# ktzsh/object-tracking

Measured on AMD Instinct MI355X. Metric: frames/sec detect+track @416x416, higher is better.
Workload: dtype f32; 1 GPU; BASELINE.json configs[2]: MultiObjDetTracker (YOLOv2 C=12 + ConvLSTM2D(512) + 1x1 + decode/NMS + track ids), 48 clips x 30 frames per GPU per step, 416x416 uint8; the synthetic head is calibrated to 32 CANDIDATE boxes per frame, of which about 20 survive NMS (config.boxes_per_frame: measured).  The step computes the model's TRACKING output, the one MultiObjDetTracker.predict reads (MultiObjDetTrac; parallelism=clip-shard x1

## Files before the change

object_tracking_amd/csrc/dt_internal.h:

```cpp
#pragma once
#include <hip/hip_runtime.h>

#include <atomic>
#include <cstdint>
#include <cstdio>
#include <map>
#include <mutex>
#include <functional>
#include <string>
#include <type_traits>
#include <vector>

#include "../../include/mi355_dt.h"

struct PerDeviceOnce {
    std::atomic<unsigned long long> mask{0};
    std::mutex mu;
    template <class F> int ensure(int *dev_out, F &&setup)
    {
        int dev = -1;
        if (hipGetDevice(&dev) != hipSuccess || dev < 0 || dev > 63) return 1;
        if (dev_out) *dev_out = dev;
        if ((mask.load(std::memory_order_acquire) >> dev) & 1ull) return 0;
        std::lock_guard<std::mutex> lk(mu);
        if ((mask.load(std::memory_order_acquire) >> dev) & 1ull) return 0;
        const int rc = setup(dev);
        if (rc == 0) mask.fetch_or(1ull << dev, std::memory_order_release);
        return rc;
    }
};

typedef float f32x4 __attribute__((ext_vector_type(4)));
typedef float f32x16 __attribute__((ext_vector_type(16)));

enum { ORD_LINEAR = 0, ORD_QUAD = 1 };
enum { EPI_PLAIN = 0, EPI_POOL = 1, EPI_POOL_BOTH = 2, EPI_S2D = 3, EPI_GATES = 4, EPI_PARTIAL = 5 };

struct ConvArgs {
    const float *in;
    long long in_bs;
    int in_ld;
    const float *wt;
    const float *bias;
    float *out;
    long long out_bs;
    int out_ld;
    float *out2;
    int out2_ld;
    const float *xproj;
    long long xp_bs;
    int xp_ld;
    float *cstate;
    long long c_bs;
    int c_ld;
    int B, H, W, Cin, N, M, K;
    int npad;
    float slope;
    int act;
    const float *zeros;
    int ksplit;
    int tile_gn;
    int zbatch;
    long long z_in, z_wt, z_out;
    int force_cfg;
    unsigned *amax_out;
};

enum { CFG_128x128 = 0, CFG_128x64 = 1, CFG_256x128 = 2, CFG_256x256 = 3, CFG_64x128 = 4 };

int launch_conv_igemm(hipStream_t st, const ConvArgs &a, int ks, int order, int epi, int cfg);
int launch_splitk_reduce(hipStream_t st, const float *slab, int S, long long M, int N, const float *bias, float slope,
                         float *out, int out_ld);

void pack_conv_weights(const float *hwio, int ks, int cin_src, int cout_src, const int *cin_map,
                       int cin_dst, const int *n_map, int npad, const float *scale, float *dst);

struct WinoArgs {
    int B, H, W, th, tw, Mt, ts;
    int g;
    const float *in;
    long long in_bs;
    int in_ld, C;
    float *v;
    unsigned short *v_s3;
    int Mp;
    int nt;
    const unsigned *amax;
    unsigned *amax_out;
    const float *m;
    int m_ld, N;
    const float *bias;
    const float *bias16;
    float slope;
    float *out;
    long long out_bs;
    int out_ld;
    float *out2;
    int out2_ld;
    const float *xproj;
    long long xp_bs;
    int xp_ld;
    float *cstate;
    long long c_bs;
    int c_ld;
};
struct Wino4FusedArgs {
    const float *in;
    long long in_bs;
    int in_ld;
    int B, H, W, Cin, N;
    const float *u;
    const float *bias;
    float slope;
    float *out;
    long long out_bs;
    int out_ld;
    float *out2;
    int out2_ld;
    int nby, nbx;
    const float *zeros;
    unsigned *amax_out;
};
int launch_wino4s_fused(hipStream_t st, const Wino4FusedArgs &a, const float *zeros);
void wino4s_fused_pack(const float *u36, int npad, int cin, int cout, float *dst);
struct Conv3H2Args {
    const float *in;
    long long in_bs;
    int in_ld;
    int B, H, W, Cin, N, Np;
    const unsigned short *w;
    const float *pscale;
    const unsigned *amax;
    const float *bias;
    float slope;
    float *out;
    long long out_bs;
    int out_ld;
    float *out2;
    int out2_ld;
    const float *zeros;
    unsigned *amax_out;
    int tiles_x, tiles_y;
    const unsigned short *w1;
    const float *pscale1;
    const float *bias1;
    int N1, Np1;
    float slope1;
};
int launch_conv3_h2(hipStream_t st, const Conv3H2Args &a);
bool conv3_h2_usable(const Conv3H2Args &a);
double conv3_h2_flops(const Conv3H2Args &a);
struct GemmS3Args {
    const unsigned short *a;
    const float *a_f32;
    int a_ld;
    const unsigned short *b;
    float *c;
    long long c_ps;
    int P, Mt, Mp, N, Np, K, ldc;
    const unsigned short *ones, *bias_s3;
    int act;
    float slope;
// ... 329 lines not shown
```

object_tracking_amd/csrc/network.hip:

```cpp
#include <algorithm>
#include <cmath>
#include <cstdarg>
#include <cstdlib>
#include <cstring>
#include <thread>

#include "dt_internal.h"

static const float BN_EPS = 1e-3f;
static const float LEAKY = 0.1f;
static char g_static_err[512] = "";

static const int TRUNK[20][5] = {
    {1, 3, 3, 32, 1},      {2, 3, 32, 64, 1},     {3, 3, 64, 128, 0},    {4, 1, 128, 64, 0},
    {5, 3, 64, 128, 1},    {6, 3, 128, 256, 0},   {7, 1, 256, 128, 0},   {8, 3, 128, 256, 1},
    {9, 3, 256, 512, 0},   {10, 1, 512, 256, 0},  {11, 3, 256, 512, 0},  {12, 1, 512, 256, 0},
    {13, 3, 256, 512, 1},  {14, 3, 512, 1024, 0}, {15, 1, 1024, 512, 0}, {16, 3, 512, 1024, 0},
    {17, 1, 1024, 512, 0}, {18, 3, 512, 1024, 0}, {19, 3, 1024, 1024, 0}, {20, 3, 1024, 1024, 0}};

static inline int round_up(int v, int m) { return (v + m - 1) / m * m; }

int dt_fail(dt_ctx *ctx, int code, const char *fmt, ...)
{
    char buf[512];
// ... 681 lines not shown
    }
    if (consumed) *consumed = off;
    graphs_clear(ctx);
    ctx->det_loaded = true;
    if (const int rc = streams_fresh(ctx)) return rc;
    return build_merged_xproj(ctx);
}

enum { DF_IGEMM = 0, DF_FUSED = 1, DF_S3 = 2, DF_CONV1 = 3, DF_C3H2 = 4 };
static const char *const k_direct_form[] = {"conv_direct_form", "conv_direct_form_fused", "conv_direct_form_s3", "conv_direct_form_conv1", "conv_direct_form_c3h2"};
static void prof_direct_form(dt_ctx *ctx, double flops, double bytes, int family = DF_IGEMM)
{
    if (!ctx->prof) return;
    ProfEntry &e = ctx->prof_tab[k_direct_form[family]];
    e.flops += flops;
    e.bytes += bytes;
}

static const int S3_MINK = 128;
static const long long C3H2_MIN_BLOCKS = 1024;

static bool wino_runs(const dt_ctx *ctx, const WinoWeights &wts, int B, int H, int W, int N)
{
    if (!wts.u) return false;
    const int ts = wts.ts, cin = wts.cin;
    const long long mt = (long long)B * ((H + ts - 1) / ts) * ((W + ts - 1) / ts);
    if (mt >= (1ll << 31) / 64) return false;
    if (4.0 * (ts + 2) * (ts + 2) * (double)mt * ((double)cin + N) > ctx->pol.wino_ws_gb * 1e9) return false;
    const int mint = ctx->pol.wino_mint;
    return ctx->pol.wino == 2 || mt >= (mint > 0 ? mint : (ts == 2 ? 256 : (ts == 4 ? 16 : 32)));
}

static double small_gemm_cost(int Mt, int N, int P, int *cfg_out)
{
    const long long t128 = (long long)P * ((Mt + 127) / 128) * ((N + 127) / 128);
    const long long t64n = (long long)P * ((Mt + 127) / 128) * ((N + 63) / 64);
    const long long t64m = (long long)P * ((Mt + 63) / 64) * ((N + 127) / 128);
    const long long t256 = (long long)P * ((Mt + 255) / 256) * ((N + 255) / 256);
    double best = (double)((t128 + 255) / 256);
    int cfg = CFG_128x128;
    const double c64n = N % 64 == 0 ? (double)((t64n + 255) / 256) * 0.5 / 0.92 : 1e30;
    const double c64m = (double)((t64m + 255) / 256) * 0.5 / 0.92;
    const double c256 = N % 256 == 0 ? (double)((t256 + 255) / 256) * 4.0 / 1.03 : 1e30;
    if (c64n < best) { best = c64n; cfg = CFG_128x64; }
    if (c64m < best) { best = c64m; cfg = CFG_64x128; }
    if (c256 < best) { best = c256; cfg = CFG_256x256; }
    if (cfg_out) *cfg_out = cfg;
    return best;
}

static int pick_cfg_gemm(int Mt, int N, int P)
{
    const long long t128 = (long long)P * ((Mt + 127) / 128) * ((N + 127) / 128);
    if (t128 <= 4096) {
        int cfg;
        (void)small_gemm_cost(Mt, N, P, &cfg);
        return cfg;
    }
    if (N % 256 == 0) {
        const long long t256 = (long long)P * ((Mt + 255) / 256) * (N / 256);
        const double e256 = (double)Mt / (((Mt + 255) / 256) * 256.0) * (double)t256 / (double)(((t256 + 255) / 256) * 256);
        const double e128 = (double)Mt / (((Mt + 127) / 128) * 128.0) * (double)t128 / (double)(((t128 + 511) / 512) * 512);
        if (e256 * 1.03 > e128) return CFG_256x256;
    }
    return CFG_128x128;
}

static int launch_igemm(dt_ctx *ctx, ConvArgs &a, int ks, int order, int epi, int cfg)
{
    a.force_cfg = ctx->pol.conv_cfg >= 0 ? ctx->pol.conv_cfg + 1 : 0;
    return launch_conv_igemm(ctx->stream, a, ks, order, epi, cfg);
}

struct WinoIO {
    const float *in; long long in_bs; int in_ld;
    float *out; long long out_bs; int out_ld;
    float *out2; int out2_ld;
    const float *xproj; long long xp_bs; int xp_ld;
    float *cstate; long long c_bs; int c_ld;
    const float *bias16;
    unsigned *amax_out;
};

struct WinoGeom { int g, th, tw, Mt; };
static WinoGeom wino_geometry(const dt_ctx *ctx, int ts, int B, int H, int W, bool pooled)
{
    WinoGeom q;
    q.g = 1;
    const int g_env = ctx->pol.mosaic;
    double best = (double)((H + ts - 1) / ts) * ((W + ts - 1) / ts);
    for (int g = 2; g <= 4 && !pooled && g_env != 1; ++g) {
        const double t = (double)((g * (H + 1) + ts - 1) / ts) * ((g * (W + 1) + ts - 1) / ts) / (g * g);
        if ((t < best * 0.97 && B >= g * g) || g_env == g) { best = t; q.g = g; }
    }
    if (q.g == 1) { q.th = (H + ts - 1) / ts; q.tw = (W + ts - 1) / ts; q.Mt = B * q.th * q.tw; }
    else {
        q.th = (q.g * (H + 1) + ts - 1) / ts; q.tw = (q.g * (W + 1) + ts - 1) / ts;
        q.Mt = ((B + q.g * q.g - 1) / (q.g * q.g)) * q.th * q.tw;
    }
    return q;
}

struct Leaves { const float *lo[2]; long long floats[2]; int next, cols; };
static Leaves conv_leaves(int epi, const float *out, int out_ld, const float *out2, int out2_ld, long long M, int cout)
{
    return Leaves{{out, out2}, {(epi == EPI_POOL || epi == EPI_S2D ? M / 4 : M) * out_ld, out2 ? M / 4 * out2_ld : 0}, epi == EPI_POOL_BOTH ? 1 : 0,
                  epi == EPI_S2D ? 4 * cout : cout};
}
static void amax_forget(dt_ctx *ctx, const Leaves &lv) { amax_forget(ctx, lv.lo[0], lv.floats[0]); amax_forget(ctx, lv.lo[1], lv.floats[1]); }
static void amax_note(dt_ctx *ctx, const Leaves &lv, int slot) { amax_note(ctx, lv.lo[lv.next], lv.floats[lv.next], lv.cols, slot); }

struct WinoChoice { WinoGeom q; int nt; };
static WinoChoice choose_wino(const dt_ctx *ctx, const WinoWeights &wts, int N, int B, int H, int W, bool pooled, bool gates)
{
    const int ts = wts.ts, cin = wts.cin;
    WinoChoice c{wino_geometry(ctx, ts, B, H, W, pooled), 0};
    const bool rec = ts == 4 && gates;
    const bool h2_avail = h2_wanted(ctx) && wts.h2;
    const int minrows = h2_avail ? ctx->pol.s3_minrows_h2 : ctx->pol.s3_minrows, rec_minrows = h2_avail ? ctx->pol.s3_rec_minrows_h2 : ctx->pol.s3_rec_minrows;
    if (((ts == 6 && !gates) || rec) && ctx->pol.s3 != 0 && cin % 32 == 0 && N % 128 == 0 && wts.npad % 128 == 0 && wino_gemm_s3_usable(c.q.Mt, cin, N) &&
        (ctx->pol.s3 == 2 || (cin >= S3_MINK && (rec ? (rec_minrows > 0 && c.q.Mt >= rec_minrows) : c.q.Mt >= minrows))) && wts.s3)
        c.nt = h2_avail ? 2 : 3;
    return c;
}
static WinoChoice choose_wino(const dt_ctx *ctx, const WinoWeights &wts, int N, int B, int H, int W, const WinoIO &io) { return choose_wino(ctx, wts, N, B, H, W, io.out2 != nullptr, io.cstate != nullptr); }

static int run_wino(dt_ctx *ctx, const WinoWeights &wts, const WinoChoice &wc, const float *bias, int N, int B, int H, int W, const WinoIO &io, float slope,
                    const char *tag, int cin_alg = 0 ,
                    int in_slot = AMAX_TEST )
{
    const int ts = wts.ts, cin = wts.cin, npad = wts.npad;
    const double cin_df = cin_alg > 0 ? cin_alg : cin;
    amax_forget(ctx, io.out ? conv_leaves(io.out2 ? EPI_POOL_BOTH : EPI_PLAIN, io.out, io.out_ld, io.out2, io.out2_ld, (long long)B * H * W, N)
                            : conv_leaves(EPI_POOL, io.out2, io.out2_ld, nullptr, 0, (long long)B * H * W, N));
    WinoArgs w{};
    w.B = B; w.H = H; w.W = W; w.ts = ts;
    w.g = wc.q.g; w.th = wc.q.th; w.tw = wc.q.tw; w.Mt = wc.q.Mt;
    prof_count(ctx, "wino_mosaic:g%d_ts%d", w.g, ts);
    const int P = (ts + 2) * (ts + 2);
    const size_t mt = (size_t)w.Mt;
    const bool h2 = wc.nt == 2;
    const unsigned short *u_s3 = h2 ? wts.h2.get() : (wc.nt == 3 ? wts.s3.get() : nullptr);
    const int NT = h2 ? 2 : 3;
    const size_t mp = (mt + 255) / 256 * 256;
    float *V = ws_get(ctx, "wino_v", u_s3 ? (size_t)P * NT * mp * cin * sizeof(unsigned short) : P * mt * cin * sizeof(float));
    float *Mp = ws_get(ctx, "wino_m", P * mt * N * sizeof(float));
    if (!V || !Mp) return DT_ERR_DEVICE;
    if (u_s3) { w.v_s3 = reinterpret_cast<unsigned short *>(V); w.Mp = (int)mp; }
    const unsigned *amax = nullptr;
    if (h2) {
        amax = in_slot == AMAX_ONE ? amax_slot(ctx, AMAX_ONE) : ensure_amax(ctx, io.in, (long long)B * H * W, cin, io.in_ld, in_slot);
        if (!amax) return DT_ERR_DEVICE;
        w.nt = 2; w.amax = amax;
    }
    w.in = io.in; w.in_bs = io.in_bs; w.in_ld = io.in_ld; w.C = cin; w.v = V;
    w.m = Mp; w.m_ld = N; w.N = N; w.bias = bias; w.bias16 = io.bias16; w.slope = slope;
    w.out = io.out; w.out_bs = io.out_bs; w.out_ld = io.out_ld; w.out2 = io.out2; w.out2_ld = io.out2_ld;
    w.xproj = io.xproj; w.xp_bs = io.xp_bs; w.xp_ld = io.xp_ld;
    w.cstate = io.cstate; w.c_bs = io.c_bs; w.c_ld = io.c_ld;
    {
        ProfScope ps(ctx, "wino_input", 0.0, 4.0 * (double)B * H * W * cin + (u_s3 ? 2.0 * NT : 4.0) * (double)P * mt * cin, tag);
        const int rc = launch_wino_input(ctx->stream, w);
        if (rc) return dt_fail(ctx, launch_code(rc), "%s: Winograd input transform launch failed", tag);
    }
    const double df_flops = 2.0 * B * H * W * 9.0 * cin_df * N;
    const double df_bytes = 4.0 * ((double)B * H * W * cin_df + 9.0 * cin_df * N + (io.out ? (double)B * H * W * N : 0.0) +
                                   (io.out2 ? (double)B * H * W * N / 4.0 : 0.0) + (io.cstate ? 4.0 * B * H * W * N / 4.0 : 0.0));
    if (u_s3) {
        GemmS3Args g{};
        g.a = w.v_s3; g.b = u_s3; g.c = Mp; g.c_ps = (long long)mt * N; g.P = P; g.Mt = w.Mt; g.Mp = (int)mp; g.N = N; g.Np = npad;
        g.K = cin; g.ldc = N; g.half = ctx->pol.s3_half;
        if (h2) { g.nt = 2; g.pscale = wts.h2_pscale.get(); g.amax = amax; }
        ProfScope ps(ctx, "conv_gemm_s3", wino_gemm_s3_flops(g), (double)P * (2.0 * NT * mt * cin + 2.0 * NT * (double)cin * N + 4.0 * (double)mt * N), tag);
        prof_count(ctx, h2 ? "s3_form:f16x2" : "s3_form:bf16x3");
        prof_direct_form(ctx, df_flops, df_bytes, DF_S3);
        if (ps.on) prof_count(ctx, wino_gemm_s3_half_chosen(g, 0) ? "s3_tile:128x2" : "s3_tile:256");
        const int rc = launch_wino_gemm_s3(ctx->stream, g, 0);
        if (rc) return dt_fail(ctx, launch_code(rc), "%s: split-bf16 Winograd GEMM launch failed (rc=%d)", tag, rc);
    } else {
        ConvArgs a{};
        a.in = V; a.in_ld = cin; a.in_bs = (long long)mt * cin;
        a.wt = wts.u.get(); a.bias = nullptr;
        a.out = Mp; a.out_ld = N; a.out_bs = (long long)mt * N;
        a.B = 1; a.H = 1; a.W = w.Mt; a.Cin = cin; a.N = N; a.M = w.Mt; a.K = cin;
        a.npad = npad; a.slope = 1.0f;
        a.zbatch = P; a.z_in = (long long)mt * cin; a.z_wt = (long long)npad * cin; a.z_out = (long long)mt * N;
        ProfScope ps(ctx, "conv_igemm", 2.0 * P * mt * (double)cin * N, 4.0 * P * ((double)mt * cin + (double)cin * N + (double)mt * N), tag);
        prof_direct_form(ctx, df_flops, df_bytes);
        const int rc = launch_igemm(ctx, a, 1, ORD_LINEAR, EPI_PLAIN, pick_cfg_gemm(w.Mt, N, P));
        if (rc) return dt_fail(ctx, launch_code(rc), "%s: Winograd GEMM launch failed (rc=%d)", tag, rc);
    }
    {
        const double outb = (io.out ? (double)B * H * W * N : 0.0) + (io.out2 ? (double)B * H * W * N / 4.0 : 0.0) +
                            (io.cstate ? 3.0 * B * H * W * N / 4.0 + (double)B * H * W * N : 0.0);
        ProfScope ps(ctx, "wino_output", 0.0, 4.0 * ((double)P * mt * N + outb), tag);
        w.amax_out = io.amax_out;
        if (!wino_output_fills_amax(w, io.cstate != nullptr)) w.amax_out = nullptr;
        const int rc = launch_wino_output(ctx->stream, w, io.cstate != nullptr);
        if (rc) return dt_fail(ctx, launch_code(rc), "%s: Winograd output transform launch failed", tag);
    }
    return DT_OK;
}

struct Dest { float *p; int ld; };

static int pick_cfg(int M, int cout, int ks)
{
    if (cout <= 64) return CFG_128x64;
    if (ks == 3 && cout % 256 == 0) {
        const long long t256 = (long long)((M + 255) / 256) * (cout / 256);
        const long long t128 = (long long)((M + 127) / 128) * (cout / 128);
        const double e256 = (double)t256 / (double)(((t256 + 255) / 256) * 256);
        const double e128 = (double)t128 / (double)(((t128 + 511) / 512) * 512);
        if (e256 * 1.05 > e128) return CFG_256x256;
    }
    if (ks == 1 && cout >= 128 && (long long)((M + 255) / 256) * ((cout + 127) / 128) >= 4096) return CFG_256x128;
    return CFG_128x128;
}

static bool s3_1x1_eligible(const dt_ctx *ctx, const ConvLayer &L, long long M)
// ... 1307 lines not shown
```

object_tracking_amd/csrc/winograd.hip:

```cpp
#include <thread>

#include "dt_internal.h"

#define WINO_THREADS 256

template <int V> struct VecOf;
template <> struct VecOf<1> { typedef float T; };
template <> struct VecOf<2> { typedef float T __attribute__((ext_vector_type(2))); };
template <> struct VecOf<4> { typedef float T __attribute__((ext_vector_type(4))); };

template <int V> __device__ __forceinline__ typename VecOf<V>::T vload(const float *p)
{
    return *reinterpret_cast<const typename VecOf<V>::T *>(p);
}
template <int V> __device__ __forceinline__ void vstore(float *p, typename VecOf<V>::T v)
{
    *reinterpret_cast<typename VecOf<V>::T *>(p) = v;
}
template <int V> __device__ __forceinline__ typename VecOf<V>::T vload_nt(const float *p)
{
    return __builtin_nontemporal_load(reinterpret_cast<const typename VecOf<V>::T *>(p));
}
template <int V> __device__ __forceinline__ void vstore_nt(float *p, typename VecOf<V>::T v)
{
    __builtin_nontemporal_store(v, reinterpret_cast<typename VecOf<V>::T *>(p));
}
template <int V> __device__ __forceinline__ float lane_of(const typename VecOf<V>::T &v, int e) { return v[e]; }
template <> __device__ __forceinline__ float lane_of<1>(const float &v, int) { return v; }
template <int V> __device__ __forceinline__ void set_lane(typename VecOf<V>::T &v, int e, float x) { v[e] = x; }
template <> __device__ __forceinline__ void set_lane<1>(float &v, int, float x) { v = x; }
template <int V> __device__ __forceinline__ typename VecOf<V>::T vzero()
{
    typename VecOf<V>::T z;
#pragma unroll
    for (int e = 0; e < V; ++e) set_lane<V>(z, e, 0.0f);
    return z;
}

template <int TS, typename T> __device__ __forceinline__ void bt_1d(T *d)
{
    if (TS == 2) {
        const T t0 = d[0] - d[2], t1 = d[1] + d[2], t2 = d[2] - d[1], t3 = d[1] - d[3];
        d[0] = t0; d[1] = t1; d[2] = t2; d[3] = t3;
    } else if (TS == 6) {
        const T t0 = d[0] - d[6] + 5.25f * (d[4] - d[2]);
        const T t7 = d[7] - d[1] + 5.25f * (d[3] - d[5]);
        const T a = d[2] - 4.25f * d[4] + d[6], b = d[1] - 4.25f * d[3] + d[5];
        const T c = 0.25f * d[2] - 1.25f * d[4] + d[6], e = 0.5f * d[1] - 2.5f * d[3] + 2.0f * d[5];
        const T f = 4.0f * d[2] - 5.0f * d[4] + d[6], g = 2.0f * d[1] - 2.5f * d[3] + 0.5f * d[5];
        d[0] = t0; d[1] = a + b; d[2] = a - b; d[3] = c + e; d[4] = c - e; d[5] = f + g; d[6] = f - g; d[7] = t7;
    } else {
        const T t0 = 4.0f * d[0] - 5.0f * d[2] + d[4];
        const T t1 = -4.0f * (d[1] + d[2]) + d[3] + d[4];
        const T t2 = 4.0f * (d[1] - d[2]) - d[3] + d[4];
        const T t3 = 2.0f * (d[3] - d[1]) - d[2] + d[4];
        const T t4 = 2.0f * (d[1] - d[3]) - d[2] + d[4];
        const T t5 = 4.0f * d[1] - 5.0f * d[3] + d[5];
        d[0] = t0; d[1] = t1; d[2] = t2; d[3] = t3; d[4] = t4; d[5] = t5;
    }
}
template <int TS, typename T> __device__ __forceinline__ void at_1d(T *m)
{
    if (TS == 2) {
        const T y0 = m[0] + m[1] + m[2], y1 = m[1] - m[2] - m[3];
        m[0] = y0; m[1] = y1;
    } else if (TS == 6) {
        const T p1 = m[1] + m[2], q1 = m[1] - m[2], p2 = m[3] + m[4], q2 = m[3] - m[4], p3 = m[5] + m[6], q3 = m[5] - m[6];
        const T y0 = m[0] + p1 + p2 + p3;
        const T y1 = q1 + 2.0f * q2 + 0.5f * q3;
        const T y2 = p1 + 4.0f * p2 + 0.25f * p3;
        const T y3 = q1 + 8.0f * q2 + 0.125f * q3;
        const T y4 = p1 + 16.0f * p2 + 0.0625f * p3;
        const T y5 = q1 + 32.0f * q2 + 0.03125f * q3 + m[7];
        m[0] = y0; m[1] = y1; m[2] = y2; m[3] = y3; m[4] = y4; m[5] = y5;
    } else {
        const T a = m[1] + m[2], b = m[1] - m[2], c = m[3] + m[4], e = m[3] - m[4];
        const T y0 = m[0] + a + c;
        const T y1 = b + 2.0f * e;
        const T y2 = a + 4.0f * c;
        const T y3 = b + 8.0f * e + m[5];
        m[0] = y0; m[1] = y1; m[2] = y2; m[3] = y3;
    }
}

struct TileId {
    int grp, ty, tx;
};
__device__ __forceinline__ TileId tile_id(const WinoArgs &p, int tile)
{
    const int tpf = p.th * p.tw;
    TileId t;
    t.grp = tile / tpf;
    const int r = tile - t.grp * tpf;
    t.ty = r / p.tw;
    t.tx = r - t.ty * p.tw;
    return t;
}
__device__ __forceinline__ bool vpixel(const WinoArgs &p, int grp, int vh, int vw, int &b, int &h, int &w)
{
    if (vh < 0 || vw < 0) return false;
    if (p.g == 1) {
        b = grp; h = vh; w = vw;
        return vh < p.H && vw < p.W;
    }
    const int fy = vh / (p.H + 1), fx = vw / (p.W + 1);
    h = vh - fy * (p.H + 1);
    w = vw - fx * (p.W + 1);
    b = (grp * p.g + fy) * p.g + fx;
    return fy < p.g && fx < p.g && h < p.H && w < p.W && b < p.B;
}

typedef __bf16 wino_bf4 __attribute__((ext_vector_type(4)));
typedef unsigned int wino_u2 __attribute__((ext_vector_type(2)));
__device__ __forceinline__ void s3_split4(const VecOf<4>::T x, wino_u2 t[3])
{
    const wino_bf4 h = __builtin_convertvector(x, wino_bf4);
    const VecOf<4>::T r1 = x - __builtin_convertvector(h, VecOf<4>::T);
    const wino_bf4 m = __builtin_convertvector(r1, wino_bf4);
    const VecOf<4>::T r2 = r1 - __builtin_convertvector(m, VecOf<4>::T);
    const wino_bf4 l = __builtin_convertvector(r2, wino_bf4);
    t[0] = __builtin_bit_cast(wino_u2, h); t[1] = __builtin_bit_cast(wino_u2, m); t[2] = __builtin_bit_cast(wino_u2, l);
}

template <typename T> __device__ __forceinline__ void s3_store(unsigned short *p, const T &v)
{
    __builtin_nontemporal_store(v, reinterpret_cast<T *>(p));
}

typedef _Float16 wino_h4 __attribute__((ext_vector_type(4)));
__device__ __forceinline__ void h2_split4(const VecOf<4>::T x, wino_u2 t[2])
{
    const wino_h4 h = __builtin_convertvector(x, wino_h4);
    const VecOf<4>::T r = x - __builtin_convertvector(h, VecOf<4>::T);
    t[0] = __builtin_bit_cast(wino_u2, h);
    t[1] = __builtin_bit_cast(wino_u2, __builtin_convertvector(r, wino_h4));
}

template <int TS, int V, bool S3 = false> __global__ __launch_bounds__(WINO_THREADS) void wino_input_kernel(WinoArgs p)
{
    static_assert(!S3 || V == 4, "the split-bf16 store is written for float4 items");
    typedef typename VecOf<V>::T T;
    constexpr int NI = TS + 2;
    const int cq_n = p.C / V;
    const long long items = (long long)p.Mt * cq_n;
    const long long plane = (long long)p.Mt * p.C;
    for (long long it = (long long)blockIdx.x * blockDim.x + threadIdx.x; it < items;
         it += (long long)gridDim.x * blockDim.x) {
        int tile, c;
        if constexpr (S3) {
            constexpr int GPB = 16 / V;
            const long long tb = it / GPB;
            c = (int)(tb / p.Mt) * 16 + (int)(it - tb * GPB) * V;
            tile = (int)(tb % p.Mt);
        } else {
            tile = (int)(it / cq_n);
            c = (int)(it - (long long)tile * cq_n) * V;
        }
        const TileId t = tile_id(p, tile);
        T d[NI][NI];
#pragma unroll
        for (int i = 0; i < NI; ++i) {
#pragma unroll
            for (int j = 0; j < NI; ++j) {
                int b, h, w;
                const bool ok = vpixel(p, t.grp, TS * t.ty - 1 + i, TS * t.tx - 1 + j, b, h, w);
                d[i][j] = ok ? vload<V>(p.in + (long long)b * p.in_bs + (long long)(h * p.W + w) * p.in_ld + c) : vzero<V>();
            }
        }
#pragma unroll
        for (int j = 0; j < NI; ++j) {
            T col[NI];
#pragma unroll
            for (int i = 0; i < NI; ++i) col[i] = d[i][j];
            bt_1d<TS>(col);
#pragma unroll
            for (int i = 0; i < NI; ++i) d[i][j] = col[i];
        }
        if constexpr (S3) {
            const long long term = (long long)(p.C >> 4) * p.Mp * 16;
            unsigned short *dst = p.v_s3 + ((long long)(c >> 4) * p.Mp + tile) * 16 + (c & 15);
#pragma unroll
            for (int i = 0; i < NI; ++i) {
                bt_1d<TS>(d[i]);
                wino_u2 tr[NI][3];
#pragma unroll
                for (int j = 0; j < NI; ++j) s3_split4(d[i][j], tr[j]);
#pragma unroll
                for (int j = 0; j < NI; ++j)
#pragma unroll
                    for (int k = 0; k < 3; ++k) s3_store(dst + ((long long)(NI * i + j) * 3 + k) * term, tr[j][k]);
            }
        } else {
            float *dst = p.v + (long long)tile * p.C + c;
#pragma unroll
            for (int i = 0; i < NI; ++i) {
                bt_1d<TS>(d[i]);
#pragma unroll
                for (int j = 0; j < NI; ++j) vstore_nt<V>(dst + (long long)(NI * i + j) * plane, d[i][j]);
            }
        }
    }
}

__device__ __forceinline__ float wino_leaky(float v, float slope) { return v > 0.0f ? v : v * slope; }
__device__ __forceinline__ float wino_hard_sigmoid(float x)
{
    const float y = __fmaf_rn(0.2f, x, 0.5f);
    return fminf(fmaxf(y, 0.0f), 1.0f);
}

template <int TS, int V>
__device__ __forceinline__ void wino_at_m_a(const float *src, long long plane, typename VecOf<V>::T (*m)[TS + 2])
{
    typedef typename VecOf<V>::T T;
    constexpr int NI = TS + 2;
#pragma unroll
    for (int i = 0; i < NI; ++i)
#pragma unroll
        for (int j = 0; j < NI; ++j) m[i][j] = vload_nt<V>(src + (long long)(NI * i + j) * plane);
#pragma unroll
    for (int j = 0; j < NI; ++j) {
        T col[NI];
#pragma unroll
        for (int i = 0; i < NI; ++i) col[i] = m[i][j];
        at_1d<TS>(col);
#pragma unroll
        for (int i = 0; i < TS; ++i) m[i][j] = col[i];
    }
#pragma unroll
    for (int i = 0; i < TS; ++i) at_1d<TS>(m[i]);
}

__device__ __forceinline__ int wino_border_case(const WinoArgs &p, int h, int w)
{
    return (h == 0 ? 1 : 0) | (h == p.H - 1 ? 2 : 0) | (w == 0 ? 4 : 0) | (w == p.W - 1 ? 8 : 0);
}

template <int TS, int V> __global__ __launch_bounds__(WINO_THREADS) void wino_output_kernel(WinoArgs p)
{
    typedef typename VecOf<V>::T T;
    constexpr int NI = TS + 2;
    const int nq = p.N / V;
    const long long items = (long long)p.Mt * nq;
    const long long plane = (long long)p.Mt * p.m_ld;
    float am = 0.0f;
    const bool am_full = p.amax_out && !p.out2, am_pool = p.amax_out && p.out2;
    for (long long it = (long long)blockIdx.x * blockDim.x + threadIdx.x; it < items;
         it += (long long)gridDim.x * blockDim.x) {
        const int tile = (int)(it / nq);
        const int c = (int)(it - (long long)tile * nq) * V;
        const TileId t = tile_id(p, tile);
        T m[NI][NI];
        wino_at_m_a<TS, V>(p.m + (long long)tile * p.m_ld + c, plane, m);
        const T bv = p.bias ? vload<V>(p.bias + c) : vzero<V>();
#pragma unroll
        for (int i = 0; i < TS; ++i)
#pragma unroll
            for (int j = 0; j < TS; ++j) {
                T v = m[i][j] + bv;
#pragma unroll
                for (int e = 0; e < V; ++e) set_lane<V>(v, e, wino_leaky(lane_of<V>(v, e), p.slope));
                m[i][j] = v;
            }
        if (p.out) {
#pragma unroll
            for (int i = 0; i < TS; ++i)
#pragma unroll
                for (int j = 0; j < TS; ++j) {
                    int b, h, w;
                    if (vpixel(p, t.grp, TS * t.ty + i, TS * t.tx + j, b, h, w)) {
                        T v = m[i][j];
                        if (p.bias16) {
                            const int k = wino_border_case(p, h, w);
                            if (k) v = v + vload<V>(p.bias16 + (long long)k * p.N + c);
                        }
                        if (am_full) {
#pragma unroll
                            for (int e = 0; e < V; ++e) am = fmaxf(am, fabsf(lane_of<V>(v, e)));
                        }
                        vstore_nt<V>(p.out + (long long)b * p.out_bs + (long long)(h * p.W + w) * p.out_ld + c, v);
                    }
                }
        }
        if (p.out2) {
            const int H2 = p.H >> 1, W2 = p.W >> 1;
#pragma unroll
            for (int i = 0; i < TS / 2; ++i)
#pragma unroll
                for (int j = 0; j < TS / 2; ++j) {
                    const int h2 = (TS / 2) * t.ty + i, w2 = (TS / 2) * t.tx + j;
                    if (h2 < H2 && w2 < W2) {
                        T mx;
#pragma unroll
                        for (int e = 0; e < V; ++e)
                            set_lane<V>(mx, e, fmaxf(fmaxf(lane_of<V>(m[2 * i][2 * j], e), lane_of<V>(m[2 * i][2 * j + 1], e)),
                                                     fmaxf(lane_of<V>(m[2 * i + 1][2 * j], e), lane_of<V>(m[2 * i + 1][2 * j + 1], e))));
                        if (am_pool) {
#pragma unroll
                            for (int e = 0; e < V; ++e) am = fmaxf(am, fabsf(lane_of<V>(mx, e)));
                        }
                        vstore<V>(p.out2 + ((long long)(t.grp * H2 + h2) * W2 + w2) * p.out2_ld + c, mx);
                    }
                }
        }
    }
    if (p.amax_out) dt_amax_publish(p.amax_out, am);
}

template <int TS, int V> __global__ __launch_bounds__(WINO_THREADS) void wino_output_gates_kernel(WinoArgs p)
{
    typedef typename VecOf<V>::T T;
    constexpr int NI = TS + 2;
    const int U = p.N >> 2;
    const int uq = U / V;
    const long long items = (long long)p.Mt * uq;
    const long long plane = (long long)p.Mt * p.m_ld;
    for (long long it = (long long)blockIdx.x * blockDim.x + threadIdx.x; it < items;
         it += (long long)gridDim.x * blockDim.x) {
        const int tile = (int)(it / uq);
        const int jc = (int)(it - (long long)tile * uq) * V;
        const int col = (jc >> 5) * 128 + (jc & 31);
        const TileId t = tile_id(p, tile);
        T y[4][TS][TS];
#pragma unroll
        for (int g = 0; g < 4; ++g) {
            T m[NI][NI];
            wino_at_m_a<TS, V>(p.m + (long long)tile * p.m_ld + col + g * 32, plane, m);
#pragma unroll
            for (int i = 0; i < TS; ++i)
#pragma unroll
                for (int j = 0; j < TS; ++j) y[g][i][j] = m[i][j];
        }
        constexpr int RG = TS >= 4 ? TS / 2 : TS;
#pragma unroll
        for (int g = 0; g < 4; ++g)
#pragma unroll
            for (int i = 0; i < TS; ++i)
#pragma unroll
                for (int j = 0; j < TS; ++j) asm volatile("" ::"v"(y[g][i][j]));
#pragma unroll
        for (int i0 = 0; i0 < TS; i0 += RG) {
            T xz[RG][TS][4], cpv[RG][TS];
            long long cofs[RG][TS], oofs[RG][TS];
            bool ok[RG][TS];
#pragma unroll
            for (int i = 0; i < RG; ++i)
#pragma unroll
                for (int j = 0; j < TS; ++j) {
                    int b = 0, h = 0, w = 0;
                    ok[i][j] = vpixel(p, t.grp, TS * t.ty + i0 + i, TS * t.tx + j, b, h, w);
                    if (!ok[i][j]) { b = 0; h = 0; w = 0; }
                    const long long pix = h * p.W + w;
                    const float *xp = p.xproj + (long long)b * p.xp_bs + pix * p.xp_ld + col;
                    cofs[i][j] = (long long)b * p.c_bs + pix * p.c_ld + jc;
                    oofs[i][j] = (long long)b * p.out_bs + pix * p.out_ld + jc;
#pragma unroll
                    for (int g = 0; g < 4; ++g) xz[i][j][g] = vload<V>(xp + 32 * g);
                    cpv[i][j] = vload<V>(p.cstate + cofs[i][j]);
                }
#pragma unroll
            for (int i = 0; i < RG; ++i)
#pragma unroll
                for (int j = 0; j < TS; ++j) {
                    const T zi = y[0][i0 + i][j] + xz[i][j][0], zf = y[1][i0 + i][j] + xz[i][j][1];
                    const T zc = y[2][i0 + i][j] + xz[i][j][2], zo = y[3][i0 + i][j] + xz[i][j][3];
                    T cn, hn;
#pragma unroll
                    for (int e = 0; e < V; ++e) {
                        const float gi = wino_hard_sigmoid(lane_of<V>(zi, e)), gf = wino_hard_sigmoid(lane_of<V>(zf, e));
                        const float go = wino_hard_sigmoid(lane_of<V>(zo, e));
                        const float cv = gf * lane_of<V>(cpv[i][j], e) + gi * tanhf(lane_of<V>(zc, e));
                        set_lane<V>(cn, e, cv);
                        set_lane<V>(hn, e, go * tanhf(cv));
                    }
                    if (ok[i][j]) {
                        vstore<V>(p.cstate + cofs[i][j], cn);
                        vstore<V>(p.out + oofs[i][j], hn);
                    }
                }
        }
    }
}

static unsigned wino_threads(long long items) { return items < 512ll * WINO_THREADS ? 64u : (unsigned)WINO_THREADS; }
static unsigned wino_blocks(long long items)
{
// ... 126 lines not shown
                } else {
                    s3_split4(ca[j], ta);
                    s3_split4(cb[j], tb);
                }
#pragma unroll
                for (int k = 0; k < NT; ++k) o[j][k] = wino_u4{ta[k][0], ta[k][1], tb[k][0], tb[k][1]};
            }
            __builtin_amdgcn_sched_barrier(0);
#pragma unroll
            for (int j = 0; j < NI; ++j)
#pragma unroll
                for (int k = 0; k < NT; ++k) s3_store(dst + ((long long)(NI * sub + j) * NT + k) * term, o[j][k]);
        }
        if constexpr (ONE) wino_item_sync(); else __syncthreads();
    }
}

__global__ __launch_bounds__(WINO_THREADS) void wino_output_coop6_kernel(WinoArgs p)
{
    typedef VecOf<4>::T T;
    __shared__ __attribute__((aligned(16))) float s_t[(WINO_THREADS / 8) * WINO_COOP_ITEM];
    const int nq = p.N / 4;
    const long long items = (long long)p.Mt * nq;
    const long long plane = (long long)p.Mt * p.m_ld;
    const int sub = threadIdx.x & 7, slot = threadIdx.x >> 3;
    float *st = s_t + slot * WINO_COOP_ITEM;
    float am = 0.0f;
    const bool am_full = p.amax_out && !p.out2, am_pool = p.amax_out && p.out2;
    for (long long base = (long long)blockIdx.x * (WINO_THREADS / 8); base < items; base += (long long)gridDim.x * (WINO_THREADS / 8)) {
        const long long it = base + slot;
        const bool live = it < items;
        const int tile = live ? (int)(it / nq) : 0;
        const int c = live ? (int)(it - (long long)tile * nq) * 4 : 0;
        const TileId t = tile_id(p, tile);
        T col[8];
        const float *src = p.m + (long long)tile * p.m_ld + c;
        T bv = vzero<4>();
        if (p.bias) bv = vload<4>(p.bias + c);
#pragma unroll
        for (int i = 0; i < 8; ++i)
            col[i] = live ? vload_nt<4>(src + (long long)(8 * i + sub) * plane) : vzero<4>();
        at_1d<6>(col);
        asm volatile("" ::"v"(bv));
#pragma unroll
        for (int i = 0; i < 6; ++i) vstore<4>(st + (sub * 9 + i) * 4, col[i]);
        wino_item_sync();
        T row[8];
#pragma unroll
        for (int j = 0; j < 8; ++j) row[j] = vzero<4>();
        if (sub < 6) {
#pragma unroll
            for (int j = 0; j < 8; ++j) row[j] = vload<4>(st + (j * 9 + sub) * 4);
            at_1d<6>(row);
#pragma unroll
            for (int j = 0; j < 6; ++j) {
                T v = row[j] + bv;
#pragma unroll
                for (int e = 0; e < 4; ++e) set_lane<4>(v, e, wino_leaky(lane_of<4>(v, e), p.slope));
                row[j] = v;
                int b, h, w;
                if (live && p.out && vpixel(p, t.grp, 6 * t.ty + sub, 6 * t.tx + j, b, h, w)) {
                    if (p.bias16) {
                        const int k = wino_border_case(p, h, w);
                        if (k) v = v + vload<4>(p.bias16 + (long long)k * p.N + c);
                    }
                    if (am_full) {
#pragma unroll
                        for (int e = 0; e < 4; ++e) am = fmaxf(am, fabsf(lane_of<4>(v, e)));
                    }
                    vstore_nt<4>(p.out + (long long)b * p.out_bs + (long long)(h * p.W + w) * p.out_ld + c, v);
                }
            }
        }
        if (p.out2) {
            const int H2 = p.H >> 1, W2 = p.W >> 1;
#pragma unroll
            for (int k = 0; k < 3; ++k) {
                T mx;
#pragma unroll
                for (int e = 0; e < 4; ++e) {
                    const float a = fmaxf(lane_of<4>(row[2 * k], e), lane_of<4>(row[2 * k + 1], e));
                    set_lane<4>(mx, e, fmaxf(a, __shfl_xor(a, 1)));
                }
                const int h2 = 3 * t.ty + (sub >> 1), w2 = 3 * t.tx + k;
                if (live && sub < 6 && !(sub & 1) && h2 < H2 && w2 < W2) {
                    if (am_pool) {
#pragma unroll
                        for (int e = 0; e < 4; ++e) am = fmaxf(am, fabsf(lane_of<4>(mx, e)));
                    }
                    vstore<4>(p.out2 + ((long long)(t.grp * H2 + h2) * W2 + w2) * p.out2_ld + c, mx);
                }
            }
        }
        wino_item_sync();
    }
    if (p.amax_out) dt_amax_publish(p.amax_out, am);
}

__global__ __launch_bounds__(256) void wino_s3_pack_kernel(const float *u, int P, int npad, int K, unsigned short *dst)
{
    const int kq = K / 4;
    const long long n_items = (long long)P * npad * kq;
    const long long term = (long long)(K >> 4) * npad * 16;
    for (long long it = (long long)blockIdx.x * blockDim.x + threadIdx.x; it < n_items; it += (long long)gridDim.x * blockDim.x) {
        const int k = (int)(it % kq) * 4;
        const long long r = it / kq;
        const int n = (int)(r % npad), pz = (int)(r / npad);
        wino_u2 tr[3];
        s3_split4(vload<4>(u + r * K + k), tr);
#pragma unroll
        for (int t3 = 0; t3 < 3; ++t3)
            *reinterpret_cast<wino_u2 *>(dst + ((long long)pz * 3 + t3) * term + ((long long)(k >> 4) * npad + n) * 16 + (k & 15)) = tr[t3];
    }
}
int launch_wino_s3_pack(hipStream_t st, const float *u, int P, int npad, int K, unsigned short *dst)
{
    if (!u || !dst || P <= 0 || npad <= 0 || K % 16) return 2;
    const long long n_items = (long long)P * npad * (K / 4);
    long long nb = (n_items + 255) / 256;
    if (nb > 65536) nb = 65536;
    hipLaunchKernelGGL(wino_s3_pack_kernel, dim3((unsigned)nb), dim3(256), 0, st, u, P, npad, K, dst);
    return hipGetLastError() == hipSuccess ? 0 : 1;
}

__global__ __launch_bounds__(256) void absmax_kernel(const float *x, long long rows, int cols, long long ld, long long plane, unsigned *slots)
{
    const float *xz = x + (long long)blockIdx.y * plane;
    const int cq = cols >> 2;
    const long long items = rows * cq;
    float m = 0.0f;
    for (long long it = (long long)blockIdx.x * blockDim.x + threadIdx.x; it < items; it += (long long)gridDim.x * blockDim.x) {
        const long long r = it / cq;
        const int c = (int)(it - r * cq) * 4;
        const VecOf<4>::T v = __builtin_nontemporal_load(reinterpret_cast<const VecOf<4>::T *>(xz + r * ld + c));
#pragma unroll
        for (int e = 0; e < 4; ++e) m = fmaxf(m, fabsf(v[e]));
    }
    if ((cols & 3) && blockIdx.x == 0)
        for (long long r = threadIdx.x; r < rows; r += blockDim.x)
            for (int c = cq * 4; c < cols; ++c) m = fmaxf(m, fabsf(xz[r * ld + c]));
    dt_amax_publish(slots + (long long)blockIdx.y * DT_AMAX_WORDS, m);
}
int launch_absmax(hipStream_t st, const float *x, long long rows, int cols, long long ld, int planes, long long plane_stride, unsigned *slots, bool zero)
{
    if (!x || !slots || rows <= 0 || cols <= 0 || planes <= 0 || planes > 65535) return 2;
    if (cols >= 4 && ((ld & 3) || (plane_stride & 3) || (reinterpret_cast<uintptr_t>(x) & 15))) return 2;
    if (zero && hipMemsetAsync(slots, 0, (size_t)planes * DT_AMAX_WORDS * sizeof(unsigned), st) != hipSuccess) return 1;
    const long long items = rows * (cols >= 4 ? cols >> 2 : 1);
    long long nb = (items + 255) / 256 / 8;
    nb = nb < 1 ? 1 : (nb > 4096 ? 4096 : nb);
    hipLaunchKernelGGL(absmax_kernel, dim3((unsigned)nb, (unsigned)planes), dim3(256), 0, st, x, rows, cols, ld, plane_stride, slots);
    return hipGetLastError() == hipSuccess ? 0 : 1;
}
__global__ __launch_bounds__(256) void wino_h2_pack_kernel(const float *u, int P, int npad, int K, const unsigned *slots, int slot_stride, unsigned short *dst)
{
    const int kq = K / 4;
    const long long n_items = (long long)P * npad * kq;
    const long long term = (long long)(K >> 4) * npad * 16;
    for (long long it = (long long)blockIdx.x * blockDim.x + threadIdx.x; it < n_items; it += (long long)gridDim.x * blockDim.x) {
        const int k = (int)(it % kq) * 4;
        const long long r = it / kq;
        const int n = (int)(r % npad), pz = (int)(r / npad);
        unsigned am = 0;
#pragma unroll
        for (int q = 0; q < DT_AMAX_SUB; ++q) { const unsigned w = slots[pz * slot_stride + q * DT_AMAX_LINE]; am = w > am ? w : am; }
        wino_u2 tr[2];
        h2_split4(vload<4>(u + r * K + k) * dt_h2_base(am), tr);
#pragma unroll
        for (int t2 = 0; t2 < 2; ++t2)
            *reinterpret_cast<wino_u2 *>(dst + ((long long)pz * 2 + t2) * term + ((long long)(k >> 4) * npad + n) * 16 + (k & 15)) = tr[t2];
    }
}
__global__ void wino_h2_pscale_kernel(const unsigned *slots, int P, int ts, float *pscale)
{
    const int p = blockIdx.x * blockDim.x + threadIdx.x;
    if (p >= P) return;
    unsigned am = 0;
    for (int q = 0; q < DT_AMAX_SUB; ++q) { const unsigned w = slots[p * DT_AMAX_WORDS + q * DT_AMAX_LINE]; am = w > am ? w : am; }
    const int ni = ts + 2;
    const float rf = ts ? dt_h2_rowfac(ts, p / ni) * dt_h2_rowfac(ts, p % ni) : 1.0f;
    pscale[p] = dt_h2_base_inv(am) / rf;
}
int launch_wino_h2_pack(hipStream_t st, const float *u, int P, int npad, int K, int ts, unsigned *slots, unsigned short *dst, float *pscale)
{
    if (!u || !dst || !slots || P <= 0 || npad <= 0 || K % 16) return 2;
    if (int rc = pscale ? launch_absmax(st, u, npad, K, K, P, (long long)npad * K, slots) : launch_absmax(st, u, (long long)P * npad, K, K, 1, 0, slots)) return rc;
    const long long n_items = (long long)P * npad * (K / 4);
    long long nb = (n_items + 255) / 256;
    if (nb > 65536) nb = 65536;
    hipLaunchKernelGGL(wino_h2_pack_kernel, dim3((unsigned)nb), dim3(256), 0, st, u, P, npad, K, slots, pscale ? DT_AMAX_WORDS : 0, dst);
    if (pscale) hipLaunchKernelGGL(wino_h2_pscale_kernel, dim3((P + 63) / 64), dim3(64), 0, st, slots, P, ts, pscale);
    return hipGetLastError() == hipSuccess ? 0 : 1;
}

static inline bool wino_coop_wanted(long long items_pairs) { return items_pairs < (long long)WINO_COOP_MAX_ITEMS; }

int launch_wino_input(hipStream_t st, const WinoArgs &a)
{
    if (a.C % 4 || a.in_ld % 4 || a.Mt <= 0 || (a.ts != 2 && a.ts != 4 && a.ts != 6) || a.g < 1) return 2;
    if (a.v_s3 && a.nt == 2) {
        if ((a.ts != 6 && a.ts != 4) || a.C % 32 || a.Mp < a.Mt || !a.amax) return 2;
        const long long wgs = ((long long)((a.Mt + 3) & ~3) * (a.C / 8) + WINO_S3IN_THREADS / 8 - 1) / (WINO_S3IN_THREADS / 8);
        const long long cap = 24576;
        const unsigned grid = (unsigned)(wgs < cap ? wgs : cap);
        if (a.ts == 6) hipLaunchKernelGGL((wino_input_s3_kernel<6, 2>), dim3(grid), dim3(WINO_S3IN_THREADS), 0, st, a);
        else hipLaunchKernelGGL((wino_input_s3_kernel<4, 2>), dim3(grid), dim3(WINO_S3IN_THREADS), 0, st, a);
    } else if (a.v_s3 && a.ts == 4) {
        if (a.C % 16 || a.Mp < a.Mt) return 2;
        if (a.C % 32 == 0) {
            const long long wgs = ((long long)((a.Mt + 3) & ~3) * (a.C / 8) + WINO_S3IN_THREADS / 8 - 1) / (WINO_S3IN_THREADS / 8);
            hipLaunchKernelGGL(wino_input_s3_kernel<4>, dim3((unsigned)(wgs < 262144 ? wgs : 262144)), dim3(WINO_S3IN_THREADS), 0, st, a);
        } else
            hipLaunchKernelGGL((wino_input_kernel<4, 4, true>), dim3(wino_blocks((long long)a.Mt * (a.C / 4))), dim3(wino_threads((long long)a.Mt * (a.C / 4))), 0, st, a);
    } else if (a.v_s3) {
        if (a.ts != 6 || a.C % 32 || a.Mp < a.Mt) return 2;
        const long long wgs = ((long long)((a.Mt + 3) & ~3) * (a.C / 8) + WINO_S3IN_THREADS / 8 - 1) / (WINO_S3IN_THREADS / 8);
        hipLaunchKernelGGL(wino_input_s3_kernel<6>, dim3((unsigned)(wgs < 262144 ? wgs : 262144)), dim3(WINO_S3IN_THREADS), 0, st, a);
    } else if (a.ts == 6 && wino_coop_wanted((long long)a.Mt * (a.C / 2))) {
        const long long wgs = ((long long)a.Mt * (a.C / 4) + WINO_THREADS / 8 - 1) / (WINO_THREADS / 8);
        hipLaunchKernelGGL(wino_input_coop6_kernel, dim3((unsigned)(wgs < 65536 ? wgs : 65536)), dim3(WINO_THREADS), 0, st, a);
    } else if (a.ts == 6)
        hipLaunchKernelGGL((wino_input_kernel<6, 2>), dim3(wino_blocks((long long)a.Mt * (a.C / 2))), dim3(wino_threads((long long)a.Mt * (a.C / 2))), 0,
                           st, a);
    else if (a.ts == 2)
        hipLaunchKernelGGL((wino_input_kernel<2, 4>), dim3(wino_blocks((long long)a.Mt * (a.C / 4))), dim3(wino_threads((long long)a.Mt * (a.C / 4))), 0,
                           st, a);
    else
        hipLaunchKernelGGL((wino_input_kernel<4, 4>), dim3(wino_blocks((long long)a.Mt * (a.C / 4))), dim3(wino_threads((long long)a.Mt * (a.C / 4))), 0,
                           st, a);
    return hipGetLastError() == hipSuccess ? 0 : 1;
}

bool wino_output_fills_amax(const WinoArgs &a, int gates)
{
    return !gates && a.amax_out != nullptr;
}
int launch_wino_output(hipStream_t st, const WinoArgs &a, int gates)
{
    if (a.m_ld % 4 || a.Mt <= 0 || (a.ts != 2 && a.ts != 4 && a.ts != 6) || a.g < 1 || (a.out2 && a.g != 1)) return 2;
    if (gates) {
        if (a.N % 128 || a.out_ld % 4 || a.c_ld % 4 || a.xp_ld % 4) return 2;
        if (a.ts == 6)
            hipLaunchKernelGGL((wino_output_gates_kernel<6, 1>), dim3(wino_blocks((long long)a.Mt * (a.N / 4))), dim3(wino_threads((long long)a.Mt * (a.N / 4))), 0, st, a);
        else if (a.ts == 2)
            hipLaunchKernelGGL((wino_output_gates_kernel<2, 4>), dim3(wino_blocks((long long)a.Mt * (a.N / 16))), dim3(wino_threads((long long)a.Mt * (a.N / 16))), 0, st, a);
        else
            hipLaunchKernelGGL((wino_output_gates_kernel<4, 1>), dim3(wino_blocks((long long)a.Mt * (a.N / 4))), dim3(wino_threads((long long)a.Mt * (a.N / 4))), 0, st, a);
    } else {
        if (a.N % 4 || (a.out && a.out_ld % 4) || (a.out2 && a.out2_ld % 4)) return 2;
        if (a.bias16 && (a.slope != 1.0f || a.out2 || !a.out)) return 2;
        if (a.ts == 6 && wino_coop_wanted((long long)a.Mt * (a.N / 2))) {
            const long long wgs = ((long long)a.Mt * (a.N / 4) + WINO_THREADS / 8 - 1) / (WINO_THREADS / 8);
            hipLaunchKernelGGL(wino_output_coop6_kernel, dim3((unsigned)(wgs < 65536 ? wgs : 65536)), dim3(WINO_THREADS), 0, st, a);
        } else if (a.ts == 6)
            hipLaunchKernelGGL((wino_output_kernel<6, 2>), dim3(wino_blocks((long long)a.Mt * (a.N / 2))), dim3(wino_threads((long long)a.Mt * (a.N / 2))),
                               0, st, a);
        else if (a.ts == 2)
            hipLaunchKernelGGL((wino_output_kernel<2, 4>), dim3(wino_blocks((long long)a.Mt * (a.N / 4))), dim3(wino_threads((long long)a.Mt * (a.N / 4))),
                               0, st, a);
        else
            hipLaunchKernelGGL((wino_output_kernel<4, 2>), dim3(wino_blocks((long long)a.Mt * (a.N / 2))), dim3(wino_threads((long long)a.Mt * (a.N / 2))),
                               0, st, a);
    }
    return hipGetLastError() == hipSuccess ? 0 : 1;
}

void wino_pack_weights(int ts, const float *hwio, int cin_src, int cout_src, const int *cin_map, int cin_dst,
                       const int *n_map, int npad, const float *scale, float *dst)
{
    static const double G2[4][3] = {{1, 0, 0}, {.5, .5, .5}, {.5, -.5, .5}, {0, 0, 1}};
    static const double G4[6][3] = {{1. / 4, 0, 0},          {-1. / 6, -1. / 6, -1. / 6}, {-1. / 6, 1. / 6, -1. / 6},
                                    {1. / 24, 1. / 12, 1. / 6}, {1. / 24, -1. / 12, 1. / 6}, {0, 0, 1}};
    static const double G6[8][3] = {{1, 0, 0},
                                    {-2. / 9, -2. / 9, -2. / 9},   {-2. / 9, 2. / 9, -2. / 9},
                                    {1. / 90, 1. / 45, 2. / 45},   {1. / 90, -1. / 45, 2. / 45},
                                    {32. / 45, 16. / 45, 8. / 45}, {32. / 45, -16. / 45, 8. / 45},
                                    {0, 0, 1}};
    const int ni = ts + 2, P = ni * ni;
    const double(*G)[3] = ts == 2 ? G2 : (ts == 4 ? G4 : G6);
    const size_t plane = (size_t)npad * cin_dst;
    auto work = [&](int n_lo, int n_hi) {
        for (int n = n_lo; n < n_hi; ++n) {
            const int ns = n_map ? n_map[n] : (n < cout_src ? n : -1);
            for (int ci = 0; ci < cin_dst; ++ci) {
                const int cs = cin_map ? cin_map[ci] : (ci < cin_src ? ci : -1);
                float *o = dst + (size_t)n * cin_dst + ci;
                if (ns < 0 || cs < 0) {
                    for (int q = 0; q < P; ++q) o[q * plane] = 0.0f;
                    continue;
                }
                const double sc = scale ? (double)scale[ns] : 1.0;
                double g[3][3], t[8][3];
                for (int k = 0; k < 9; ++k) g[k / 3][k % 3] = (double)hwio[((size_t)k * cin_src + cs) * cout_src + ns] * sc;
                for (int xi = 0; xi < ni; ++xi)
                    for (int kx = 0; kx < 3; ++kx) t[xi][kx] = G[xi][0] * g[0][kx] + G[xi][1] * g[1][kx] + G[xi][2] * g[2][kx];
                for (int xi = 0; xi < ni; ++xi)
                    for (int nu = 0; nu < ni; ++nu)
                        o[(size_t)(ni * xi + nu) * plane] = (float)(t[xi][0] * G[nu][0] + t[xi][1] * G[nu][1] + t[xi][2] * G[nu][2]);
            }
        }
    };
    const int nthreads = npad >= 64 ? 8 : 1;
    std::vector<std::thread> pool;
    for (int i = 0; i < nthreads; ++i)
        pool.emplace_back(work, (int)((long long)npad * i / nthreads), (int)((long long)npad * (i + 1) / nthreads));
    for (auto &th : pool) th.join();
}
```

Before: 16970 frames/s.

## Extend Winograd mosaic tiling to pooled convs and larger grid factors

Winograd mosaic packing, which lays several images into one padded canvas to cut wasted tile area, was previously disabled for convs with a fused max-pool output and capped at a 4x4 grid. This adds per-image pitch fields (padded to even sizes when pooling), allows grid factors up to 6, and rewrites the output kernels to walk mosaic coordinates incrementally and scatter pooled outputs to the correct image. The aim is fewer padded tiles on small feature maps, at the cost of extra per-pixel bounds logic in the output kernels and less tile-count gain from the larger even padding.

```diff
diff --git a/object_tracking_amd/csrc/dt_internal.h b/object_tracking_amd/csrc/dt_internal.h
--- a/object_tracking_amd/csrc/dt_internal.h
+++ b/object_tracking_amd/csrc/dt_internal.h
@@ -78,6 +78,7 @@
 struct WinoArgs {
     int B, H, W, th, tw, Mt, ts;
     int g;
+    int ph, pw;
     const float *in;
     long long in_bs;
     int in_ld, C;
diff --git a/object_tracking_amd/csrc/network.hip b/object_tracking_amd/csrc/network.hip
--- a/object_tracking_amd/csrc/network.hip
+++ b/object_tracking_amd/csrc/network.hip
@@ -787,20 +787,22 @@
     unsigned *amax_out;
 };
 
-struct WinoGeom { int g, th, tw, Mt; };
+struct WinoGeom { int g, ph, pw, th, tw, Mt; };
 static WinoGeom wino_geometry(const dt_ctx *ctx, int ts, int B, int H, int W, bool pooled)
 {
     WinoGeom q;
     q.g = 1;
+    q.ph = pooled ? (H + 2) & ~1 : H + 1;
+    q.pw = pooled ? (W + 2) & ~1 : W + 1;
     const int g_env = ctx->pol.mosaic;
     double best = (double)((H + ts - 1) / ts) * ((W + ts - 1) / ts);
-    for (int g = 2; g <= 4 && !pooled && g_env != 1; ++g) {
-        const double t = (double)((g * (H + 1) + ts - 1) / ts) * ((g * (W + 1) + ts - 1) / ts) / (g * g);
+    for (int g = 2; g <= 6 && g_env != 1; ++g) {
+        const double t = (double)((g * q.ph + ts - 1) / ts) * ((g * q.pw + ts - 1) / ts) / (g * g);
         if ((t < best * 0.97 && B >= g * g) || g_env == g) { best = t; q.g = g; }
     }
     if (q.g == 1) { q.th = (H + ts - 1) / ts; q.tw = (W + ts - 1) / ts; q.Mt = B * q.th * q.tw; }
     else {
-        q.th = (q.g * (H + 1) + ts - 1) / ts; q.tw = (q.g * (W + 1) + ts - 1) / ts;
+        q.th = (q.g * q.ph + ts - 1) / ts; q.tw = (q.g * q.pw + ts - 1) / ts;
         q.Mt = ((B + q.g * q.g - 1) / (q.g * q.g)) * q.th * q.tw;
     }
     return q;
@@ -840,7 +842,7 @@
                             : conv_leaves(EPI_POOL, io.out2, io.out2_ld, nullptr, 0, (long long)B * H * W, N));
     WinoArgs w{};
     w.B = B; w.H = H; w.W = W; w.ts = ts;
-    w.g = wc.q.g; w.th = wc.q.th; w.tw = wc.q.tw; w.Mt = wc.q.Mt;
+    w.g = wc.q.g; w.ph = wc.q.ph; w.pw = wc.q.pw; w.th = wc.q.th; w.tw = wc.q.tw; w.Mt = wc.q.Mt;
     prof_count(ctx, "wino_mosaic:g%d_ts%d", w.g, ts);
     const int P = (ts + 2) * (ts + 2);
     const size_t mt = (size_t)w.Mt;
diff --git a/object_tracking_amd/csrc/winograd.hip b/object_tracking_amd/csrc/winograd.hip
--- a/object_tracking_amd/csrc/winograd.hip
+++ b/object_tracking_amd/csrc/winograd.hip
@@ -103,9 +103,43 @@
         b = grp; h = vh; w = vw;
         return vh < p.H && vw < p.W;
     }
-    const int fy = vh / (p.H + 1), fx = vw / (p.W + 1);
-    h = vh - fy * (p.H + 1);
-    w = vw - fx * (p.W + 1);
+    const int fy = vh / p.ph, fx = vw / p.pw;
+    h = vh - fy * p.ph;
+    w = vw - fx * p.pw;
+    b = (grp * p.g + fy) * p.g + fx;
+    return fy < p.g && fx < p.g && h < p.H && w < p.W && b < p.B;
+}
+__device__ __forceinline__ bool pooled_pixel(const WinoArgs &p, int grp, int vh, int vw, int &b, int &h2, int &w2)
+{
+    int h = 0, w = 0;
+    const bool ok = vpixel(p, grp, vh, vw, b, h, w);
+    h2 = h >> 1; w2 = w >> 1;
+    return ok && h2 < (p.H >> 1) && w2 < (p.W >> 1);
+}
+struct TileOrg {
+    int fy, h, fx, w;
+    int ph, pw;
+};
+template <int TS> __device__ __forceinline__ TileOrg tile_org(const WinoArgs &p, const TileId &t)
+{
+    TileOrg o;
+    if (p.g == 1) {
+        o.fy = 0; o.h = TS * t.ty; o.fx = 0; o.w = TS * t.tx;
+        o.ph = o.pw = 0x7fffffff;
+    } else {
+        o.fy = TS * t.ty / p.ph; o.h = TS * t.ty - o.fy * p.ph;
+        o.fx = TS * t.tx / p.pw; o.w = TS * t.tx - o.fx * p.pw;
+        o.ph = p.ph; o.pw = p.pw;
+    }
+    return o;
+}
+__device__ __forceinline__ void mosaic_step(int &f, int &x, int pitch, int d)
+{
+    x += d;
+    if (x >= pitch) { x -= pitch; ++f; }
+}
+__device__ __forceinline__ bool mosaic_pixel(const WinoArgs &p, int grp, int fy, int h, int fx, int w, int &b)
+{
     b = (grp * p.g + fy) * p.g + fx;
     return fy < p.g && fx < p.g && h < p.H && w < p.W && b < p.B;
 }
@@ -250,6 +284,7 @@
         const int tile = (int)(it / nq);
         const int c = (int)(it - (long long)tile * nq) * V;
         const TileId t = tile_id(p, tile);
+        const TileOrg o = tile_org<TS>(p, t);
         T m[NI][NI];
         wino_at_m_a<TS, V>(p.m + (long long)tile * p.m_ld + c, plane, m);
         const T bv = p.bias ? vload<V>(p.bias + c) : vzero<V>();
@@ -263,12 +298,14 @@
                 m[i][j] = v;
             }
         if (p.out) {
-#pragma unroll
-            for (int i = 0; i < TS; ++i)
+            int fy = o.fy, h = o.h;
+#pragma unroll
+            for (int i = 0; i < TS; ++i) {
+                int fx = o.fx, w = o.w;
 #pragma unroll
                 for (int j = 0; j < TS; ++j) {
-                    int b, h, w;
-                    if (vpixel(p, t.grp, TS * t.ty + i, TS * t.tx + j, b, h, w)) {
+                    int b;
+                    if (mosaic_pixel(p, t.grp, fy, h, fx, w, b)) {
                         T v = m[i][j];
                         if (p.bias16) {
                             const int k = wino_border_case(p, h, w);
@@ -280,16 +317,22 @@
                         }
                         vstore_nt<V>(p.out + (long long)b * p.out_bs + (long long)(h * p.W + w) * p.out_ld + c, v);
                     }
+                    mosaic_step(fx, w, o.pw, 1);
                 }
+                mosaic_step(fy, h, o.ph, 1);
+            }
         }
         if (p.out2) {
             const int H2 = p.H >> 1, W2 = p.W >> 1;
-#pragma unroll
-            for (int i = 0; i < TS / 2; ++i)
+            int fy = o.fy, h = o.h;
+#pragma unroll
+            for (int i = 0; i < TS / 2; ++i) {
+                int fx = o.fx, w = o.w;
 #pragma unroll
                 for (int j = 0; j < TS / 2; ++j) {
-                    const int h2 = (TS / 2) * t.ty + i, w2 = (TS / 2) * t.tx + j;
-                    if (h2 < H2 && w2 < W2) {
+                    int b;
+                    const int h2 = h >> 1, w2 = w >> 1;
+                    if (mosaic_pixel(p, t.grp, fy, h, fx, w, b) && h2 < H2 && w2 < W2) {
                         T mx;
 #pragma unroll
                         for (int e = 0; e < V; ++e)
@@ -299,9 +342,12 @@
 #pragma unroll
                             for (int e = 0; e < V; ++e) am = fmaxf(am, fabsf(lane_of<V>(mx, e)));
                         }
-                        vstore<V>(p.out2 + ((long long)(t.grp * H2 + h2) * W2 + w2) * p.out2_ld + c, mx);
+                        vstore<V>(p.out2 + (((long long)b * H2 + h2) * W2 + w2) * p.out2_ld + c, mx);
                     }
+                    mosaic_step(fx, w, o.pw, 2);
                 }
+                mosaic_step(fy, h, o.ph, 2);
+            }
         }
     }
     if (p.amax_out) dt_amax_publish(p.amax_out, am);
@@ -594,13 +640,13 @@
                     const float a = fmaxf(lane_of<4>(row[2 * k], e), lane_of<4>(row[2 * k + 1], e));
                     set_lane<4>(mx, e, fmaxf(a, __shfl_xor(a, 1)));
                 }
-                const int h2 = 3 * t.ty + (sub >> 1), w2 = 3 * t.tx + k;
-                if (live && sub < 6 && !(sub & 1) && h2 < H2 && w2 < W2) {
+                int b, h2, w2;
+                if (live && sub < 6 && !(sub & 1) && pooled_pixel(p, t.grp, 6 * t.ty + sub, 6 * t.tx + 2 * k, b, h2, w2)) {
                     if (am_pool) {
 #pragma unroll
                         for (int e = 0; e < 4; ++e) am = fmaxf(am, fabsf(lane_of<4>(mx, e)));
                     }
-                    vstore<4>(p.out2 + ((long long)(t.grp * H2 + h2) * W2 + w2) * p.out2_ld + c, mx);
+                    vstore<4>(p.out2 + (((long long)b * H2 + h2) * W2 + w2) * p.out2_ld + c, mx);
                 }
             }
         }
@@ -707,9 +753,16 @@
 
 static inline bool wino_coop_wanted(long long items_pairs) { return items_pairs < (long long)WINO_COOP_MAX_ITEMS; }
 
+static inline bool wino_pitch_ok(const WinoArgs &a)
+{
+    if (a.g < 1) return false;
+    if (a.g == 1) return true;
+    return a.ph > a.H && a.pw > a.W && !(a.out2 && ((a.ph | a.pw) & 1));
+}
+
 int launch_wino_input(hipStream_t st, const WinoArgs &a)
 {
-    if (a.C % 4 || a.in_ld % 4 || a.Mt <= 0 || (a.ts != 2 && a.ts != 4 && a.ts != 6) || a.g < 1) return 2;
+    if (a.C % 4 || a.in_ld % 4 || a.Mt <= 0 || (a.ts != 2 && a.ts != 4 && a.ts != 6) || !wino_pitch_ok(a)) return 2;
     if (a.v_s3 && a.nt == 2) {
         if ((a.ts != 6 && a.ts != 4) || a.C % 32 || a.Mp < a.Mt || !a.amax) return 2;
         const long long wgs = ((long long)((a.Mt + 3) & ~3) * (a.C / 8) + WINO_S3IN_THREADS / 8 - 1) / (WINO_S3IN_THREADS / 8);
@@ -749,7 +802,7 @@
 }
 int launch_wino_output(hipStream_t st, const WinoArgs &a, int gates)
 {
-    if (a.m_ld % 4 || a.Mt <= 0 || (a.ts != 2 && a.ts != 4 && a.ts != 6) || a.g < 1 || (a.out2 && a.g != 1)) return 2;
+    if (a.m_ld % 4 || a.Mt <= 0 || (a.ts != 2 && a.ts != 4 && a.ts != 6) || !wino_pitch_ok(a)) return 2;
     if (gates) {
         if (a.N % 128 || a.out_ld % 4 || a.c_ld % 4 || a.xp_ld % 4) return 2;
         if (a.ts == 6)
```

After: 17160 frames/s, median of 6. +1.1%, better.
